# dpeerlab/sctools

Hardware: AMD Instinct MI355X
Metric: Hamming pair-comparisons/sec, 737K 10x whitelist all-pairs, 1-8 GPUs (higher is better)
Workload: dtype i32; 1 GPU; config 2: 737280-barcode all-pairs TwoBit Hamming histogram + summary; barcodes=737280, barcode_length=16, pairs=271790530560, scheme=spectral, parallelism=single GPU

## Files before the change

sctools_amd/csrc/spectral.hip:

```cpp
#include <string.h>

#include <algorithm>
#include <vector>
#include <type_traits>

#include <mutex>

#include <hipcub/hipcub.hpp>

#include "sct_common.h"
#include "spectral.h"
#include "spectral_seed.h"
#ifdef SCT_SEED_MX_VARIANT
#include "spectral_seed_mx.h"
#endif

namespace sct_spectral {
namespace {

using Cols = Columns<kLoBits>;
constexpr int kLo = Cols::kLo;
constexpr int kHiBits = Cols::kHiBits;
constexpr int kRegGroups = 2;
constexpr int kMaxOrder = 1 << 16;

template <int N>
__device__ __forceinline__ void wht(int32_t* x) {
#pragma unroll
  for (int h = 1; h < N; h <<= 1)
#pragma unroll
    for (int i = 0; i < N; ++i)
      if (!(i & h)) {
        const int32_t a = x[i], b = x[i | h];
        x[i] = a + b;
        x[i | h] = a - b;
      }
}

constexpr int kSortWGs = 128;
constexpr int kSortThreads = 1024;

__global__ __launch_bounds__(kSortThreads) void column_hist_wg_kernel(const uint64_t* __restrict__ codes, int64_t n,
                                                                      uint32_t* __restrict__ H) {
  __shared__ uint32_t h[kLo];
  for (int c = threadIdx.x; c < kLo; c += kSortThreads) h[c] = 0;
  __syncthreads();
  int64_t b, e;
  wg_range(n, b, e);
  for (int64_t i = b + threadIdx.x; i < e; i += kSortThreads) atomicAdd(&h[codes[i] & (kLo - 1)], 1u);
  __syncthreads();
  uint32_t* out = H + (int64_t)blockIdx.x * kLo;
  for (int c = threadIdx.x; c < kLo; c += kSortThreads) out[c] = h[c];
}

__global__ __launch_bounds__(256) void column_prefix_kernel(uint32_t* __restrict__ H, int wgs,
                                                            uint32_t* __restrict__ m) {
  const int c = blockIdx.x * 256 + threadIdx.x;
  uint32_t run = 0;
#pragma unroll 8
  for (int g = 0; g < wgs; ++g) {
    const uint32_t v = H[(int64_t)g * kLo + c];
    H[(int64_t)g * kLo + c] = run;
    run += v;
  }
  m[c] = run;
}

__global__ __launch_bounds__(1024) void column_scan16_kernel(const uint32_t* __restrict__ m,
                                                             uint32_t* __restrict__ off,
                                                             uint32_t* __restrict__ gofs) {
  __shared__ uint32_t wsum[2][16];
  const int t = threadIdx.x, lane = t & 63, wave = t >> 6;
  uint32_t v[16];
#pragma unroll
  for (int k = 0; k < 4; ++k) {
    const uint4 q = reinterpret_cast<const uint4*>(m)[t * 4 + k];
    v[4 * k] = q.x;
    v[4 * k + 1] = q.y;
    v[4 * k + 2] = q.z;
    v[4 * k + 3] = q.w;
  }
  uint32_t s = 0, sg = 0;
#pragma unroll
  for (int k = 0; k < 16; ++k) {
    s += v[k];
    sg += (v[k] + 31) / 32;
  }
  uint32_t is = s, isg = sg;
#pragma unroll
  for (int d = 1; d < 64; d <<= 1) {
    const uint32_t a = __shfl_up(is, d), ag = __shfl_up(isg, d);
    if (lane >= d) {
      is += a;
      isg += ag;
    }
  }
  if (lane == 63) {
    wsum[0][wave] = is;
    wsum[1][wave] = isg;
  }
  __syncthreads();
  uint32_t base = 0, baseg = 0;
  for (int w = 0; w < wave; ++w) {
    base += wsum[0][w];
    baseg += wsum[1][w];
  }
  uint32_t run = base + is - s, rung = baseg + isg - sg;
  uint32_t o[16], og[16];
#pragma unroll
  for (int k = 0; k < 16; ++k) {
    o[k] = run;
    og[k] = rung;
    run += v[k];
    rung += (v[k] + 31) / 32;
  }
#pragma unroll
  for (int k = 0; k < 4; ++k) {
    reinterpret_cast<uint4*>(off)[t * 4 + k] = make_uint4(o[4 * k], o[4 * k + 1], o[4 * k + 2], o[4 * k + 3]);
    reinterpret_cast<uint4*>(gofs)[t * 4 + k] = make_uint4(og[4 * k], og[4 * k + 1], og[4 * k + 2], og[4 * k + 3]);
  }
  if (t == 1023) {
    off[kLo] = run;
    gofs[kLo] = rung;
  }
}

__global__ __launch_bounds__(kSortThreads) void column_scatter_wg_kernel(const uint64_t* __restrict__ codes,
                                                                         int64_t n,
                                                                         const uint32_t* __restrict__ H,
                                                                         const uint32_t* __restrict__ off,
                                                                         uint32_t* __restrict__ hi) {
  __shared__ uint32_t cur[kLo];
  const uint32_t* pre = H + (int64_t)blockIdx.x * kLo;
  for (int c = threadIdx.x; c < kLo; c += kSortThreads) cur[c] = off[c] + pre[c];
  __syncthreads();
  int64_t b, e;
  wg_range(n, b, e);
  for (int64_t i = b + threadIdx.x; i < e; i += kSortThreads) {
    const uint64_t x = codes[i];
    hi[atomicAdd(&cur[x & (kLo - 1)], 1u)] = (uint32_t)(x >> kLoBits);
  }
}

__global__ void planes_kernel(const uint32_t* __restrict__ hi, const uint32_t* __restrict__ off,
                              const uint32_t* __restrict__ gofs, int64_t max_groups,
                              uint32_t* __restrict__ planes) {
  const int64_t g = blockIdx.x * (int64_t)blockDim.x + threadIdx.x;
  if (g >= (int64_t)gofs[kLo]) return;
  int a = 0, b = kLo;
  while (b - a > 1) {
    const int m = (a + b) >> 1;
    if (gofs[m] <= (uint32_t)g) a = m;
    else b = m;
  }
  const uint32_t first = off[a] + 32u * ((uint32_t)g - gofs[a]);
  const uint32_t last = min(first + 32u, off[a + 1]);
  uint32_t p[kHiBits];
#pragma unroll
  for (int k = 0; k < kHiBits; ++k) p[k] = 0;
  for (uint32_t i = first; i < last; ++i) {
    const uint32_t h = hi[i], bit = 1u << (i - first);
#pragma unroll
    for (int k = 0; k < kHiBits; ++k) p[k] |= (h >> k) & 1u ? bit : 0u;
  }
  store_planes<Cols>(planes, g, p);
}

typedef unsigned v4u __attribute__((ext_vector_type(4)));

template <typename T>
struct Chunk {
  static constexpr int kVals = 16 / sizeof(T);
  static constexpr int kLog = sizeof(T) == 1 ? 4 : (sizeof(T) == 2 ? 3 : 2);
  static constexpr int kPerThread = 64 / kVals;
};

template <typename T>
__device__ __forceinline__ int column_pos(int c) {
  constexpr int L = Chunk<T>::kLog;
  return (c & ((1 << L) - 1)) | (((c >> 4) & 255) << L) | (((c >> L) & ((16 >> L) - 1)) << (L + 8)) |
         ((c >> 12) << 12);
}


template <typename T>
__device__ __forceinline__ void seed_body(const uint32_t* __restrict__ planes, const uint32_t* __restrict__ gofs,
                                          const uint32_t* __restrict__ off, int z0, int z1, T* __restrict__ buf) {
  constexpr int NT = 256;
  constexpr int P = 4 / sizeof(T);
  constexpr int V = Chunk<T>::kVals;
  __shared__ uint32_t stage[(kWalk / P) * NT];
  const int tid = threadIdx.x;
  const int c0 = blockIdx.x * NT, c = c0 + tid;
  const int m = (int)(off[c + 1] - off[c]);
  const uint32_t g0 = gofs[c];
  const int ng = (int)(gofs[c + 1] - g0);
  int wng = ng;
#pragma unroll
  for (int s = 32; s; s >>= 1) wng = max(wng, __shfl_xor(wng, s));
  uint32_t pr[kRegGroups][kHiBits];
#pragma unroll
  for (int g = 0; g < kRegGroups; ++g)
    if (g < ng) {
      load_planes<Cols>(planes, (int64_t)g0 + g, pr[g]);
    } else {
#pragma unroll
      for (int k = 0; k < kHiBits; ++k) pr[g][k] = 0u;
    }
  {
    const int ph = (blockIdx.x + blockIdx.y) % 3;
    if (ph >= 1) __builtin_amdgcn_s_sleep(24);
    if (ph == 2) __builtin_amdgcn_s_sleep(24);
  }
  const int za = z0 & ~(kWalk - 1);
  const int nwalks = (z1 - za + kWalk - 1) / kWalk;
  for (int wk = blockIdx.y; wk < nwalks; wk += gridDim.y) {
    const int zblk = za + wk * kWalk;
    int acc[kWalk];
    auto walk = [&](const uint32_t* p, auto first) {
      uint32_t x = 0;
#pragma unroll
      for (int k = kWalkBits; k < kHiBits; ++k)
        if ((zblk >> k) & 1) x ^= p[k];
      if constexpr (decltype(first)::value) acc[0] = __popc(x);
      else acc[0] += __popc(x);
#pragma unroll
      for (int i = 1; i < kWalk; ++i) {
        x ^= p[ctz_c(i)];
        if constexpr (decltype(first)::value) acc[gray(i)] = __popc(x);
        else acc[gray(i)] += __popc(x);
      }
    };
    walk(pr[0], std::true_type());
#pragma unroll
    for (int g = 1; g < kRegGroups; ++g)
      if (g < wng) walk(pr[g], std::false_type());
    for (int g = kRegGroups; g < wng; ++g) {
      uint32_t p[kHiBits];
      if (g < ng) {
        load_planes<Cols>(planes, (int64_t)g0 + g, p);
      } else {
#pragma unroll
        for (int k = 0; k < kHiBits; ++k) p[k] = 0u;
      }
      walk(p, std::false_type());
    }
    {
      __syncthreads();
      auto sidx = [](int row, int col) { return row * 256 + (col ^ (((col >> 6) & 3) << 2)); };
#pragma unroll
      for (int r = 0; r < kWalk / P; ++r) {
        uint32_t w = 0;
#pragma unroll
        for (int j = 0; j < P; ++j)
          w |= ((uint32_t)(m - 2 * acc[r * P + j]) & (0xFFFFFFFFu >> (32 - 8 * sizeof(T)))) << (8 * sizeof(T) * j);
        stage[sidx(r, tid)] = w;
      }
      __syncthreads();
      constexpr int kBlocks = (kWalk / P) * (256 / V);
#pragma unroll
      for (int r = 0; r < kBlocks / 256; ++r) {
        const int b = tid + 256 * r, row = b / (256 / V), cb = (b % (256 / V)) * V;
        uint32_t d[V];
#pragma unroll
        for (int k = 0; k < V; k += 4) {
          const uint4 v = *reinterpret_cast<const uint4*>(stage + sidx(row, cb + k));
          d[k] = v.x;
          d[k + 1] = v.y;
          d[k + 2] = v.z;
          d[k + 3] = v.w;
        }
        uint32_t out[P][4];
        if constexpr (P == 2) {
#pragma unroll
          for (int k = 0; k < 4; ++k) {
            out[0][k] = __builtin_amdgcn_perm(d[2 * k + 1], d[2 * k], 0x05040100u);
            out[1][k] = __builtin_amdgcn_perm(d[2 * k + 1], d[2 * k], 0x07060302u);
          }
        } else {
#pragma unroll
          for (int k = 0; k < 4; ++k) out[0][k] = d[k];
        }
#pragma unroll
        for (int j = 0; j < P; ++j) {
          const int z = zblk + row * P + j;
          if (z < z0 || z >= z1) continue;
          *reinterpret_cast<uint4*>(buf + (int64_t)(z - z0) * kLo + column_pos<T>(c0 + cb)) =
              make_uint4(out[j][0], out[j][1], out[j][2], out[j][3]);
        }
      }
    }
  }
}

__global__ __launch_bounds__(256) __attribute__((amdgpu_waves_per_eu(5))) void seed_sm_kernel(
    const uint32_t* __restrict__ planes, const uint32_t* __restrict__ gofs, const uint32_t* __restrict__ off, int z0,
    int z1, int8_t* __restrict__ buf, int lp) {
  seed_sm_body<Cols>(planes, gofs, off, z0, z1, buf, lp);
}

#ifdef SCT_SEED_MX_VARIANT
__global__ __launch_bounds__(64 * kMxWaves) void seed_mx_kernel(const uint32_t* __restrict__ planes,
                                                                const uint32_t* __restrict__ gofs,
                                                                const uint32_t* __restrict__ off, int z0, int z1,
                                                                int8_t* __restrict__ buf, int sb) {
  seed_mx_body<Cols>(planes, gofs, off, z0, z1, buf, sb);
}
#endif

template <typename T>
__global__ __launch_bounds__(256) void seed_kernel(const uint32_t* __restrict__ planes,
                                                   const uint32_t* __restrict__ gofs,
                                                   const uint32_t* __restrict__ off, int z0, int z1,
                                                   T* __restrict__ buf) {
  seed_body<T>(planes, gofs, off, z0, z1, buf);
}

__device__ __forceinline__ int swz(int e) {
  return e ^ (((e >> 6) & 1) << 2) ^ (((e >> 5) & 1) << 3) ^ (((e >> 10) & 1) << 4);
}

__device__ __forceinline__ void lane_butterfly32(int32_t& a, int32_t& b) {
  const auto r = __builtin_amdgcn_permlane32_swap((unsigned)a, (unsigned)b, false, false);
  a = (int32_t)(r[0] + r[1]);
  b = (int32_t)(r[0] - r[1]);
}
__device__ __forceinline__ void lane_butterfly16(int32_t& a, int32_t& b) {
  const auto r = __builtin_amdgcn_permlane16_swap((unsigned)a, (unsigned)b, false, false);
  a = (int32_t)(r[0] + r[1]);
  b = (int32_t)(r[0] - r[1]);
}

template <typename T>
__global__ __launch_bounds__(256) void tile_kernel(const T* __restrict__ buf, int z0, int nslices,
                                                   unsigned long long* __restrict__ counts,
                                                   unsigned long long add_n,
                                                   const unsigned long long* __restrict__ sumsq) {
  static_assert(sizeof(T) >= 2, "int8 seeds take tile_reg_kernel");
  __shared__ int32_t lds[kLo];
  __shared__ unsigned long long bins_lo[17], bins_hi[17];
  constexpr int V = Chunk<T>::kVals, L = Chunk<T>::kLog;
  const int tid = threadIdx.x, lane = tid & 63, wave = tid >> 6;
  if (tid < 17) bins_lo[tid] = bins_hi[tid] = 0;
  const int t2 = (lane & 15) | ((lane >> 4) << 10) | (wave << 12);
  const int wt_thread = digit_weight((uint32_t)lane | ((uint32_t)wave << 12));
  for (int s = blockIdx.x; s < nslices; s += gridDim.x) {
    const T* row = buf + (int64_t)s * kLo;
    int32_t x[64];
#pragma unroll
    for (int j = 0; j < Chunk<T>::kPerThread; ++j) {
      const v4u v = __builtin_nontemporal_load(reinterpret_cast<const v4u*>(row + tid * V + (j << (L + 8))));
      const T* e = reinterpret_cast<const T*>(&v);
#pragma unroll
      for (int r = 0; r < V; ++r) x[j * V + r] = e[r];
    }
    wht<64>(x);
    __syncthreads();
#pragma unroll
    for (int q = 0; q < 64; q += 4)
      *reinterpret_cast<int4*>(lds + swz((q & 15) | (tid << 4) | ((q >> 4) << 12))) =
          make_int4(x[q], x[q + 1], x[q + 2], x[q + 3]);
    __syncthreads();
    const int a2 = swz(t2);
#pragma unroll
    for (int q = 0; q < 64; ++q) x[q] = lds[a2 ^ swz(q << 4)];
    wht<64>(x);
#pragma unroll
    for (int q = 0; q < 64; ++q)
      if (!(q & 2)) lane_butterfly32(x[q], x[q | 2]);
#pragma unroll
    for (int q = 0; q < 64; ++q)
      if (!(q & 1)) lane_butterfly16(x[q], x[q | 1]);
    unsigned long long acc[4] = {0, 0, 0, 0};
#pragma unroll
    for (int q = 0; q < 64; ++q)
      acc[digit_weight_c((uint32_t)(q & 3)) + digit_weight_c((uint32_t)(q >> 2))] +=
          (unsigned long long)((int64_t)x[q] * x[q]);
    const int w0 = digit_weight((uint32_t)(z0 + s)) + wt_thread;
#pragma unroll
    for (int k = 0; k < 4; ++k) {
      if (acc[k] & 0xFFFFFFFFull) atomicAdd(&bins_lo[w0 + k], acc[k] & 0xFFFFFFFFull);
      if (acc[k] >> 32) atomicAdd(&bins_hi[w0 + k], acc[k] >> 32);
    }
  }
  __syncthreads();
  if (tid < 17) add_weight_sum(counts, tid, bins_lo[tid], bins_hi[tid]);
  add_job_constants(counts, add_n, sumsq);
}

typedef int v4i_t __attribute__((ext_vector_type(4)));
typedef short v2s_t __attribute__((ext_vector_type(2)));

typedef int v16i_t __attribute__((ext_vector_type(16)));
constexpr unsigned kChainMaxM = 125;
template <bool Chain>
__global__ __launch_bounds__(256) __attribute__((amdgpu_waves_per_eu(3))) void tile_reg_kernel(
    const int8_t* __restrict__ buf, const uint16_t* __restrict__ order, int z0, int nslices,
    unsigned long long* __restrict__ counts, unsigned long long add_n, const unsigned long long* __restrict__ sumsq) {
  __shared__ unsigned long long bins[17];
  const int tid = threadIdx.x, lane = tid & 63, wave = __builtin_amdgcn_readfirstlane(tid >> 6);
  if (tid < 17) bins[tid] = 0;
  __syncthreads();
  v4i_t H[2][2];
#pragma unroll
  for (int d = 0; d < 4; ++d) {
    uint32_t v = 0;
#pragma unroll
    for (int r = 0; r < 4; ++r) {
      const int row = lane & 31, col = 16 * (lane >> 5) + 4 * d + r;
      v |= ((__popc(row & col) & 1) ? 0xFFu : 0x01u) << (8 * r);
    }
    H[0][0][d] = H[0][1][d] = H[1][0][d] = (int)v;
    H[1][1][d] = (int)(v ^ 0xFEFEFEFEu);
  }
  v4i_t H64[2][2];
  if constexpr (Chain) {
#pragma unroll
    for (int d = 0; d < 4; ++d) {
      const uint32_t v = ((uint32_t)H[0][0][d] << 6) & 0xC0C0C0C0u;
      H64[0][0][d] = H64[0][1][d] = H64[1][0][d] = (int)v;
      H64[1][1][d] = (int)(v ^ 0x80808080u);
    }
  }
  const int wt_thread = digit_weight((uint32_t)lane);
  const int lane_off = 16 * (lane >> 5) + 32 * ((lane >> 3) & 1) + 64 * (lane & 3) + 256 * ((lane >> 4) & 1) +
                       512 * ((lane >> 2) & 1);
  const int gw = blockIdx.x * 4 + wave, GW = gridDim.x * 4;
  const int ub = (int)((int64_t)nslices * gw / GW), ue = (int)((int64_t)nslices * (gw + 1) / GW);
  unsigned long long accA[4] = {0, 0, 0, 0}, accB[4] = {0, 0, 0, 0}, accB2[4] = {0, 0, 0, 0};
  int cur_w = -1;
  auto flush = [&]() {
#pragma unroll
    for (int k = 0; k < 4; ++k) {
      if (accA[k]) atomicAdd(&bins[cur_w + wt_thread + k], accA[k]);
      const unsigned long long b = 4 * (accB[k] + accB2[k]) - accA[k];
      if (b) atomicAdd(&bins[cur_w + wt_thread + k + 1], b);
      accA[k] = 0;
      accB[k] = 0;
      accB2[k] = 0;
    }
  };
  auto load_plane = [&](int sl, int R, v4i_t* dst) {
    const int8_t* p = buf + ((int64_t)sl * kLo + 4096 * R) + lane_off;
#pragma unroll
    for (int k = 0; k < 4; ++k)
      dst[k] = __builtin_nontemporal_load(reinterpret_cast<const v4i_t*>(p + 1024 * k));
  };
  auto stage2 = [&](const v4i_t* Bl, const v4i_t* Bh, auto nt_c, auto chain_c, unsigned long long* acc,
                    unsigned long long* acc2) {
    constexpr int nt = decltype(nt_c)::value;
    v16i_t c[2];
#pragma unroll
    for (int t = 0; t < 2; ++t)
#pragma unroll
      for (int i = 0; i < 16; ++i) c[t][i] = 0;
    if constexpr (decltype(chain_c)::value) {
      v4i_t Bh4[2];
#pragma unroll
      for (int ks = 0; ks < 2; ++ks)
#pragma unroll
        for (int d = 0; d < 4; ++d) Bh4[ks][d] = (int)(((uint32_t)Bh[ks][d] << 2) & 0xFCFCFCFCu);
#pragma unroll
      for (int ks = 0; ks < 2; ++ks)
#pragma unroll
        for (int t = 0; t < 2; ++t)
          c[t] = __builtin_amdgcn_mfma_i32_32x32x32_i8(H64[t][ks], Bh4[ks], c[t], 0, 0, 0);
    } else {
#pragma unroll
      for (int ks = 0; ks < 2; ++ks)
#pragma unroll
        for (int t = 0; t < 2; ++t) c[t] = __builtin_amdgcn_mfma_i32_32x32x32_i8(H[t][ks], Bh[ks], c[t], 0, 0, 0);
#pragma unroll
      for (int t = 0; t < 2; ++t)
#pragma unroll
        for (int i = 0; i < 16; ++i) c[t][i] <<= 8;
    }
#pragma unroll
    for (int ks = 0; ks < 2; ++ks)
#pragma unroll
      for (int t = 0; t < 2; ++t) c[t] = __builtin_amdgcn_mfma_i32_32x32x32_i8(H[t][ks], Bl[ks], c[t], 0, 0, 0);
#pragma unroll
    for (int i = 0; i < 16; ++i) {
      constexpr int w0 = digit_weight_c((uint32_t)nt), w1 = digit_weight_c((uint32_t)(nt | 2));
      const int wi = digit_weight_c((uint32_t)(i & 3)) + digit_weight_c((uint32_t)(i >> 2));
#ifdef SCT_TILE_SQ_ABL
      acc[wi + w0] ^= (uint32_t)c[0][i];
      acc2[wi + w1] ^= (uint32_t)c[1][i];
#else
      acc[wi + w0] += (unsigned long long)((int64_t)c[0][i] * c[0][i]);
      acc2[wi + w1] += (unsigned long long)((int64_t)c[1][i] * c[1][i]);
#endif
    }
  };
  auto split16 = [&](const uint32_t* pr, v4i_t& Bl, v4i_t& Bh) {
#pragma unroll
    for (int d = 0; d < 4; ++d) {
      Bl[d] = (int)(__builtin_amdgcn_perm(pr[2 * d + 1], pr[2 * d], 0x06040200u) ^ 0x80808080u);
      Bh[d] = (int)__builtin_amdgcn_perm(pr[2 * d + 1], pr[2 * d], 0x07050301u);
    }
  };
  auto pairs16 = [&](const v16i_t& c1, uint32_t* pr) {
#pragma unroll
    for (int k = 0; k < 8; ++k)
      pr[k] = __builtin_amdgcn_perm((uint32_t)c1[2 * k + 1], (uint32_t)c1[2 * k], 0x05040100u);
  };
  auto slice_at = [&](int u) { return order ? ((u & ~(kMaxOrder - 1)) | (int)order[u & (kMaxOrder - 1)]) : u; };
  v4i_t dn[4];
  int s_next = ub < ue ? slice_at(ub) : 0;
  if (ub < ue) load_plane(s_next, 0, dn);
  for (int u = ub; u < ue; ++u) {
    const int s = s_next;
    const bool more = u + 1 < ue;
    if (more) s_next = slice_at(u + 1);
    const int wz = digit_weight((uint32_t)(z0 + s));
    if (wz != cur_w) {
      if (cur_w >= 0) flush();
      cur_w = wz;
    }
    uint32_t csp[2][2][8];
#pragma unroll
    for (int nt = 0; nt < 2; ++nt)
#pragma unroll
      for (int mt = 0; mt < 2; ++mt)
#pragma unroll
        for (int k = 0; k < 8; ++k) csp[nt][mt][k] = 0xFE80FE80u;
#pragma unroll 1
    for (int R = 0; R < 4; ++R) {
      v4i_t d[4];
#pragma unroll
      for (int k = 0; k < 4; ++k) d[k] = dn[k];
      if (R < 3 || more) load_plane(R < 3 ? s : s_next, R < 3 ? R + 1 : 0, dn);
      auto ntile = [&](auto nt_c) {
        constexpr int nt = decltype(nt_c)::value;
        v16i_t c1[2];
#pragma unroll
        for (int mt = 0; mt < 2; ++mt)
#pragma unroll
          for (int i = 0; i < 16; ++i) c1[mt][i] = 128;
#pragma unroll
        for (int ks = 0; ks < 2; ++ks)
#pragma unroll
          for (int mt = 0; mt < 2; ++mt)
            c1[mt] = __builtin_amdgcn_mfma_i32_32x32x32_i8(d[2 * mt + ks], H[nt][ks], c1[mt], 0, 0, 0);
        v4i_t Bl[2], Bh[2];
#pragma unroll
        for (int mt = 0; mt < 2; ++mt) {
          uint32_t pr[8];
          pairs16(c1[mt], pr);
#pragma unroll
          for (int k = 0; k < 8; ++k)
            csp[nt][mt][k] = __builtin_bit_cast(uint32_t, __builtin_bit_cast(v2s_t, csp[nt][mt][k]) +
                                                              __builtin_bit_cast(v2s_t, pr[k]));
          split16(pr, Bl[mt], Bh[mt]);
        }
        stage2(Bl, Bh, nt_c, std::bool_constant<Chain>(), accB, Chain ? accB : accB2);
        __builtin_amdgcn_sched_barrier(0);
      };
      ntile(std::integral_constant<int, 0>());
      ntile(std::integral_constant<int, 1>());
    }
    v4i_t Bl[2], Bh[2];
    split16(csp[0][0], Bl[0], Bh[0]);
    split16(csp[0][1], Bl[1], Bh[1]);
    stage2(Bl, Bh, std::integral_constant<int, 0>(), std::false_type(), accA, accA);
    split16(csp[1][0], Bl[0], Bh[0]);
    split16(csp[1][1], Bl[1], Bh[1]);
    stage2(Bl, Bh, std::integral_constant<int, 1>(), std::false_type(), accA, accA);
  }
  if (cur_w >= 0) flush();
  __syncthreads();
  if (tid < 17) add_weight_sum64(counts, tid, bins[tid]);
  add_job_constants(counts, add_n, sumsq);
}

__global__ void low32_kernel(const uint64_t* __restrict__ codes, int64_t n, uint32_t* __restrict__ out) {
  for (int64_t i = blockIdx.x * (int64_t)blockDim.x + threadIdx.x; i < n; i += (int64_t)gridDim.x * blockDim.x)
    out[i] = (uint32_t)codes[i];
}

__global__ __launch_bounds__(256) void sumsq_kernel(const uint32_t* __restrict__ sorted, int64_t n,
                                                    unsigned long long* __restrict__ out) {
  unsigned long long acc = 0;
  for (int64_t i = blockIdx.x * (int64_t)blockDim.x + threadIdx.x; i < n; i += (int64_t)gridDim.x * blockDim.x) {
    const uint32_t v = sorted[i];
    int64_t r = 0;
    if (i > 0 && sorted[i - 1] == v) {
      int64_t a = 0, b = i - 1;
      while (a < b) {
        const int64_t m = (a + b) >> 1;
        if (sorted[m] < v) a = m + 1;
        else b = m;
      }
      r = i - a;
    }
    acc += 2 * (unsigned long long)r + 1;
  }
#pragma unroll
  for (int s = 32; s; s >>= 1) acc += __shfl_xor(acc, s);
  if ((threadIdx.x & 63) == 0 && acc) atomicAdd(out, acc);
}

__global__ __launch_bounds__(256) void probe_kernel(const uint64_t* __restrict__ codes, int64_t n,
                                                    uint32_t* __restrict__ cnt14, uint32_t* __restrict__ cnt16,
                                                    unsigned long long* __restrict__ out) {
  unsigned long long o = 0;
  for (int64_t i = blockIdx.x * (int64_t)blockDim.x + threadIdx.x; i < n; i += (int64_t)gridDim.x * blockDim.x) {
    const uint64_t x = codes[i];
    o |= x;
    atomicAdd(&cnt14[x & (kLo - 1)], 1u);
    atomicAdd(&cnt16[x & 0xFFFFu], 1u);
  }
#pragma unroll
  for (int s = 32; s; s >>= 1) o |= __shfl_xor(o, s);
  if ((threadIdx.x & 63) == 0 && o) atomicOr(out, o);
}
constexpr int64_t kProbeHistMin = 1 << 17;
__global__ __launch_bounds__(kSortThreads) void probe_hist14_kernel(const uint64_t* __restrict__ codes, int64_t n,
                                                                    uint32_t* __restrict__ H,
                                                                    unsigned long long* __restrict__ out) {
  __shared__ uint32_t h[kLo];
  for (int c = threadIdx.x; c < kLo; c += kSortThreads) h[c] = 0;
  __syncthreads();
  int64_t b, e;
  wg_range(n, b, e);
  unsigned long long o = 0;
  for (int64_t i = b + threadIdx.x; i < e; i += kSortThreads) {
    const uint64_t x = codes[i];
    o |= x;
    atomicAdd(&h[x & (kLo - 1)], 1u);
  }
#pragma unroll
  for (int s = 32; s; s >>= 1) o |= __shfl_xor(o, s);
  if ((threadIdx.x & 63) == 0 && o) atomicOr(out, o);
  __syncthreads();
  uint32_t* row = H + (int64_t)blockIdx.x * kLo;
  for (int c = threadIdx.x; c < kLo; c += kSortThreads) row[c] = h[c];
}

__global__ __launch_bounds__(256) void probe_max14_kernel(const uint32_t* __restrict__ H, int wgs,
                                                          unsigned long long* __restrict__ out) {
  const int c = blockIdx.x * 256 + threadIdx.x;
  uint32_t m = 0;
#pragma unroll 8
  for (int g = 0; g < wgs; ++g) m += H[(int64_t)g * kLo + c];
#pragma unroll
  for (int s = 32; s; s >>= 1) m = max(m, (uint32_t)__shfl_xor(m, s));
  if ((threadIdx.x & 63) == 0 && m) atomicMax(out + 1, (unsigned long long)m);
}

__global__ __launch_bounds__(256) void probe_max_kernel(const uint32_t* __restrict__ cnt14,
                                                        const uint32_t* __restrict__ cnt16,
                                                        unsigned long long* __restrict__ out) {
  const int c = blockIdx.x * 256 + threadIdx.x;
  unsigned m14 = c < kLo ? cnt14[c] : 0u, m16 = cnt16[c];
#pragma unroll
  for (int s = 32; s; s >>= 1) {
    m14 = max(m14, (unsigned)__shfl_xor(m14, s));
    m16 = max(m16, (unsigned)__shfl_xor(m16, s));
  }
  if ((threadIdx.x & 63) == 0) {
    if (m14) atomicMax(out + 1, (unsigned long long)m14);
    if (m16) atomicMax(out + 2, (unsigned long long)m16);
  }
}

template <typename T>
int launch_seed(State& st, T* buf, int z0, int z1, hipStream_t s) {
  if constexpr (sizeof(T) == 1) {
#ifdef SCT_SEED_MX_VARIANT
    return launch_seed_mx<Cols>(seed_mx_kernel, st, buf, z0, z1, s);
#else
    return launch_seed_sm<Cols>(seed_sm_kernel, st, buf, z0, z1, s);
#endif
  } else {
    const int walks = (z1 - (z0 & ~(kWalk - 1)) + kWalk - 1) / kWalk;
    const int per_wg = std::max(1, std::min(kSeedWalks, walks / 64));
    const dim3 sgrid(kLo / 256, (unsigned)((walks + per_wg - 1) / per_wg));
    hipLaunchKernelGGL(seed_kernel<T>, sgrid, dim3(256), 0, s, st.d_planes, st.d_gofs, st.d_off, z0, z1, buf);
    SCT_LAUNCH_CHECK();
    return SCT_OK;
  }
}

template <typename T>
int launch_tile(State& st, int z0, int z1, unsigned long long* counts, hipStream_t s, unsigned long long add_n = 0) {
  T* buf = reinterpret_cast<T*>(st.d_buf);
  if constexpr (sizeof(T) == 1) {
    const int ns = z1 - z0;
    const uint16_t* order = ((ns & (ns - 1)) == 0 && z0 % ns == 0) ? st.d_order + std::min(ns, kMaxOrder) : nullptr;
    const dim3 rgrid((unsigned)std::max(1, std::min(st.grid * st.tile_wgs, (z1 - z0 + 3) / 4)));
    hipLaunchKernelGGL(st.tile_chain ? tile_reg_kernel<true> : tile_reg_kernel<false>, rgrid, dim3(256), 0, s, buf,
                       order, z0, z1 - z0, counts, add_n, st.sumsq_ptr());
  } else {
    const dim3 grid((unsigned)std::min(st.grid * 2, z1 - z0));
    hipLaunchKernelGGL(tile_kernel<T>, grid, dim3(256), 0, s, buf, z0, z1 - z0, counts, add_n,
                       st.sumsq_ptr());
  }
  SCT_LAUNCH_CHECK();
  return SCT_OK;
}

template <typename T>
int launch_chunk(State& st, int z0, int z1, unsigned long long* counts, hipStream_t s, unsigned long long add_n) {
  return launch_seed_tile(
      st, s, [&] { return launch_seed<T>(st, reinterpret_cast<T*>(st.d_buf), z0, z1, s); },
      [&] { return launch_tile<T>(st, z0, z1, counts, s, add_n); });
}

template <typename T>
int time_chunk(State& st, int z0, int z1, unsigned long long* counts, int repeats, hipStream_t s,
               double* seed_ms, double* tile_ms) {
  return time_seed_tile(
      st, repeats, s, [&] { return launch_seed<T>(st, reinterpret_cast<T*>(st.d_buf), z0, z1, s); },
      [&] { return launch_tile<T>(st, z0, z1, counts, s); }, seed_ms, tile_ms);
}

}

struct Workspace {
  int device = -1;
  bool busy = false;
  bool release = false;
  bool order_ready = false;
  void* p[W_NSLOTS] = {};
  size_t cap[W_NSLOTS] = {};
  bool arena = false;
  uint8_t* base = nullptr;
  size_t size = 0, used = 0;
  std::vector<void*> extra;
};

namespace {
std::mutex g_ws_mu;
Workspace* g_ws[64] = {};

void ws_free(Workspace* ws) {
  if (ws->arena) {
    if (ws->base) (void)hipFree(ws->base);
    for (void* q : ws->extra) (void)hipFree(q);
  } else {
    for (int k = 0; k < W_NSLOTS; ++k)
      if (ws->p[k]) (void)hipFree(ws->p[k]);
  }
  delete ws;
}
}

Workspace* ws_arena(size_t bytes) {
  auto* ws = new Workspace();
  ws->arena = true;
  ws->busy = true;
  if (hipGetDevice(&ws->device) != hipSuccess || hipMalloc((void**)&ws->base, bytes) != hipSuccess) {
    (void)hipGetLastError();
    ws->base = nullptr;
    bytes = 0;
  }
  ws->size = bytes;
  return ws;
}

Workspace* ws_acquire() {
  if (sct::tune(SCT_TUNE_PLAN_CACHE, 1) == 0) return nullptr;
  int dev = 0;
  if (hipGetDevice(&dev) != hipSuccess || dev < 0 || dev >= 64) return nullptr;
  std::lock_guard<std::mutex> lk(g_ws_mu);
  Workspace*& ws = g_ws[dev];
  if (!ws) {
    ws = new Workspace();
    ws->device = dev;
  }
  if (ws->busy) return nullptr;
  ws->busy = true;
  ws->release = false;
  return ws;
}

void ws_release(Workspace* ws) {
  if (!ws) return;
  if (ws->arena) {
    ws_free(ws);
    return;
  }
  std::lock_guard<std::mutex> lk(g_ws_mu);
  ws->busy = false;
  if (ws->release) {
    g_ws[ws->device] = nullptr;
    ws_free(ws);
  }
}

int ws_get(Workspace* ws, int slot, size_t bytes, void** p) {
  bytes = std::max<size_t>(bytes, 256);
  if (!ws) {
    SCT_HIP(hipMalloc(p, bytes));
    return SCT_OK;
  }
  if (ws->arena) {
    if (ws->cap[slot] < bytes) {
      const size_t at = (ws->used + 255) & ~(size_t)255;
      if (ws->base && at + bytes <= ws->size) {
        ws->p[slot] = ws->base + at;
        ws->used = at + bytes;
      } else {
        void* q = nullptr;
        SCT_HIP(hipMalloc(&q, bytes));
        ws->extra.push_back(q);
        ws->p[slot] = q;
      }
      ws->cap[slot] = bytes;
      if (slot == W_ORDER) ws->order_ready = false;
    }
    *p = ws->p[slot];
    return SCT_OK;
  }
  if (ws->cap[slot] < bytes) {
    if (ws->p[slot]) (void)hipFree(ws->p[slot]);
    ws->p[slot] = nullptr;
    ws->cap[slot] = 0;
    if (slot == W_ORDER) ws->order_ready = false;
    SCT_HIP(hipMalloc(&ws->p[slot], bytes));
    ws->cap[slot] = bytes;
  }
  *p = ws->p[slot];
  return SCT_OK;
}

void ws_put(Workspace* ws, void* p) {
  if (!ws && p) (void)hipFree(p);
}

bool* ws_order_ready(Workspace* ws) { return ws ? &ws->order_ready : nullptr; }

void ws_release_all() {
  std::lock_guard<std::mutex> lk(g_ws_mu);
  for (auto& ws : g_ws) {
    if (!ws) continue;
    if (ws->busy) {
      ws->release = true;
      continue;
    }
    int cur = 0;
    const bool dev_ok = hipGetDevice(&cur) == hipSuccess && hipSetDevice(ws->device) == hipSuccess;
    ws_free(ws);
    if (dev_ok) (void)hipSetDevice(cur);
    ws = nullptr;
  }
}

void note_stream(State& st, hipStream_t s) {
  for (auto& u : st.used)
    if (u.first == s) {
      (void)hipEventRecord(u.second, s);
      return;
    }
  hipEvent_t e = nullptr;
  if (hipEventCreateWithFlags(&e, hipEventDisableTiming) != hipSuccess) return;
  (void)hipEventRecord(e, s);
  st.used.emplace_back(s, e);
}

int make_order_table(State& st) {
  static const std::vector<uint16_t> order = [] {
    std::vector<uint16_t> o(2 * kMaxOrder);
    for (int len = 1; len <= kMaxOrder; len *= 2) {
      int start[10] = {};
      for (int u = 0; u < len; ++u) ++start[digit_weight_c((uint32_t)u) + 1];
      for (int w = 1; w < 10; ++w) start[w] += start[w - 1];
      uint16_t* b = o.data() + len;
      for (int u = 0; u < len; ++u) b[start[digit_weight_c((uint32_t)u)]++] = (uint16_t)u;
    }
    return o;
  }();
  void* p = nullptr;
  if (int rc = ws_get(st.ws, W_ORDER, order.size() * 2, &p); rc != SCT_OK) return rc;
  st.d_order = reinterpret_cast<uint16_t*>(p);
  bool* ready = ws_order_ready(st.ws);
  if (!ready || !*ready) {
    SCT_HIP(hipMemcpy(st.d_order, order.data(), order.size() * 2, hipMemcpyHostToDevice));
    if (ready) *ready = true;
  }
  return SCT_OK;
}

int probe(Workspace* ws, const uint64_t* d_codes, int64_t n, unsigned long long* out) {
  void* p = nullptr;
  constexpr size_t kWords = (size_t)kLo + (1u << 16);
  const bool hist = n >= kProbeHistMin;
  const size_t hbytes = hist ? (size_t)kSortWGs * kLo * 4 : 0;
  if (int rc = ws_get(ws, W_PROBE, hbytes + kWords * 4 + 32, &p); rc != SCT_OK) return rc;
  struct Put {
    Workspace* ws;
    void* p;
    ~Put() { ws_put(ws, p); }
  } put{ws, p};
  uint32_t* H = reinterpret_cast<uint32_t*>(p);
  uint32_t* cnt14 = reinterpret_cast<uint32_t*>(reinterpret_cast<uint8_t*>(p) + hbytes);
  uint32_t* cnt16 = cnt14 + kLo;
  unsigned long long* res = reinterpret_cast<unsigned long long*>(cnt16 + (1u << 16));
  const int blocks = (int)std::max<int64_t>(1, std::min<int64_t>(1024, sct::ceil_div(n, 256)));
  if (hist) {
    SCT_HIP(hipMemsetAsync(res, 0, 32, 0));
    hipLaunchKernelGGL(probe_hist14_kernel, dim3(kSortWGs), dim3(kSortThreads), 0, 0, d_codes, n, H, res);
    SCT_LAUNCH_CHECK();
    hipLaunchKernelGGL(probe_max14_kernel, dim3(kLo / 256), dim3(256), 0, 0, H, kSortWGs, res);
    SCT_LAUNCH_CHECK();
    SCT_HIP(hipMemcpy(out, res, 3 * sizeof(unsigned long long), hipMemcpyDeviceToHost));
    if (out[1] <= 127 && sct::tune(SCT_TUNE_SPECTRAL_COLUMNS, 0) != kLoBits16) return SCT_OK;
  }
  SCT_HIP(hipMemsetAsync(cnt14, 0, kWords * 4 + 32, 0));
  if (n > 0) {
    hipLaunchKernelGGL(probe_kernel, dim3(blocks), dim3(256), 0, 0, d_codes, n, cnt14, cnt16, res);
    SCT_LAUNCH_CHECK();
    hipLaunchKernelGGL(probe_max_kernel, dim3((1u << 16) / 256), dim3(256), 0, 0, cnt14, cnt16, res);
    SCT_LAUNCH_CHECK();
  }
  SCT_HIP(hipMemcpy(out, res, 3 * sizeof(unsigned long long), hipMemcpyDeviceToHost));
  return SCT_OK;
}

int alloc_buf(State& st, int64_t* chunk, int64_t min_chunk, size_t bytes_per_slice) {
  for (;;) {
    const size_t bytes = (size_t)((*chunk + 15) & ~15ll) * bytes_per_slice;
    const int rc = ws_get(st.ws, W_BUF, bytes, &st.d_buf);
    if (rc == SCT_OK) {
      st.buf_bytes = bytes;
      return SCT_OK;
    }
    (void)hipGetLastError();
    if (rc != SCT_E_NOMEM || *chunk / 2 < min_chunk) return rc;
    *chunk /= 2;
  }
}

template <typename K>
static int tile_wgs_per_cu(K kernel) {
  int v = 0;
  if (hipOccupancyMaxActiveBlocksPerMultiprocessor(&v, kernel, 256, 0) != hipSuccess || v <= 0) v = 2;
  return v;
}

int create(State& st, const uint64_t* d_codes, int64_t n, int64_t chunk, int cus, unsigned max14, unsigned max16) {
  st.n = n;
  st.chunk = std::max<int64_t>(kWalk, std::min<int64_t>(chunk, kSlices));
  st.grid = std::max(1, cus);
  if (n < 2) return SCT_OK;
  const unsigned maxm = max14;
  const int64_t force = sct::tune(SCT_TUNE_SPECTRAL_COLUMNS, 0);
  if (((maxm > 127 && force != kLoBits) || force == kLoBits16) && max16 <= 127)
    return create16(st, d_codes, n, max16, chunk, cus);
  if (int rc = get_slot(st, W_HI, (size_t)n * 4, &st.d_hi); rc != SCT_OK) return rc;
  if (int rc = get_slot(st, W_OFF, (size_t)(kLo + 1) * 4, &st.d_off); rc != SCT_OK) return rc;
  if (int rc = get_slot(st, W_CNT, (size_t)2 * kLo * 4, &st.d_cnt); rc != SCT_OK) return rc;
  st.max_m = maxm;
  st.elem_bytes = maxm <= 127 ? 1 : (maxm <= 32767 ? 2 : 4);
  st.chunk = std::min<int64_t>(st.chunk, (int64_t(4) << 30) / ((int64_t)kLo * st.elem_bytes));
  st.tile_chain = st.elem_bytes == 1 && maxm <= kChainMaxM && sct::tune(SCT_TUNE_TILE_CHAIN, 1) != 0;
  static const int per_cu[2] = {tile_wgs_per_cu(tile_reg_kernel<false>), tile_wgs_per_cu(tile_reg_kernel<true>)};
  st.tile_wgs = per_cu[st.tile_chain];
  if (int rc = make_order_table(st); rc != SCT_OK) return rc;
  st.max_groups = sct::ceil_div(n, 32) + kLo;
  if (int rc = get_slot(st, W_GOFS, (size_t)(kLo + 1) * 4, &st.d_gofs); rc != SCT_OK) return rc;
  if (int rc = get_slot(st, W_HIST, (size_t)kSortWGs * kLo * 4, &st.d_hist); rc != SCT_OK) return rc;
  if (int rc = get_slot(st, W_PLANES, (size_t)st.max_groups * Cols::kPlaneWords * 4, &st.d_planes); rc != SCT_OK)
    return rc;
  if (int rc = alloc_buf(st, &st.chunk, std::min<int64_t>(st.chunk, 4096), (size_t)kLo * st.elem_bytes); rc != SCT_OK)
    return rc;
  if (int rc = get_slot(st, W_SUMSQ, sizeof(unsigned long long), &st.d_sumsq); rc != SCT_OK) return rc;
  return SCT_OK;
}

void wait_idle(State& st) {
  for (auto& u : st.used) {
    (void)hipEventSynchronize(u.second);
    (void)hipEventDestroy(u.second);
  }
  st.used.clear();
}

void destroy(State& st) {
  wait_idle(st);
  for (void* p : {(void*)st.d_hi, (void*)st.d_off, (void*)st.d_cnt, (void*)st.d_gofs, (void*)st.d_planes,
                  (void*)st.d_hist, st.d_buf, (void*)st.d_order, (void*)st.d_sumsq, st.d_sumsq_tmp})
    ws_put(st.ws, p);
  ws_release(st.ws);
  st = State();
}

int ensure_sumsq(State& st, const uint64_t* d_codes, hipStream_t s) {
  if (st.sumsq_ready || st.distinct) return SCT_OK;
  size_t tmp = 0;
  SCT_HIP(hipcub::DeviceRadixSort::SortKeys(nullptr, tmp, (const uint32_t*)nullptr, (uint32_t*)nullptr, (int)st.n, 0,
                                            32, s));
  const size_t keys = ((size_t)st.n * 4 + 255) & ~(size_t)255;
  const size_t need = 2 * keys + tmp;
  char* base = reinterpret_cast<char*>(st.d_buf);
  if (need > st.buf_bytes) {
    if (int rc = ws_get(st.ws, W_SUMSQ_TMP, need, &st.d_sumsq_tmp); rc != SCT_OK) return rc;
    base = reinterpret_cast<char*>(st.d_sumsq_tmp);
  }
  uint32_t* k0 = reinterpret_cast<uint32_t*>(base);
  uint32_t* k1 = reinterpret_cast<uint32_t*>(base + keys);
  const int blocks = (int)std::min<int64_t>(2048, sct::ceil_div(st.n, 256));
  hipLaunchKernelGGL(low32_kernel, dim3(blocks), dim3(256), 0, s, d_codes, st.n, k0);
  SCT_LAUNCH_CHECK();
  SCT_HIP(hipcub::DeviceRadixSort::SortKeys(base + 2 * keys, tmp, k0, k1, (int)st.n, 0, 32, s));
  SCT_HIP(hipMemsetAsync(st.d_sumsq, 0, sizeof(unsigned long long), s));
  hipLaunchKernelGGL(sumsq_kernel, dim3(blocks), dim3(256), 0, s, k1, st.n, st.d_sumsq);
  SCT_LAUNCH_CHECK();
  st.sumsq_ready = true;
  return SCT_OK;
}

int build(State& st, const uint64_t* d_codes, hipStream_t s) {
  if (st.n < 2) return SCT_OK;
  if (int rc = ensure_sumsq(st, d_codes, s); rc != SCT_OK) return rc;
  if (st.lo_bits == kLoBits16) return build16(st, d_codes, s);
  hipEvent_t t0 = st.timer ? st.timer->start(s) : nullptr;
  hipLaunchKernelGGL(column_hist_wg_kernel, dim3(kSortWGs), dim3(kSortThreads), 0, s, d_codes, st.n, st.d_hist);
  SCT_LAUNCH_CHECK();
  hipLaunchKernelGGL(column_prefix_kernel, dim3(kLo / 256), dim3(256), 0, s, st.d_hist, kSortWGs, st.d_cnt);
  SCT_LAUNCH_CHECK();
  hipLaunchKernelGGL(column_scan16_kernel, dim3(1), dim3(1024), 0, s, st.d_cnt, st.d_off, st.d_gofs);
  SCT_LAUNCH_CHECK();
  hipLaunchKernelGGL(column_scatter_wg_kernel, dim3(kSortWGs), dim3(kSortThreads), 0, s, d_codes, st.n, st.d_hist,
                     st.d_off, st.d_hi);
  SCT_LAUNCH_CHECK();
  if (st.max_m <= 32 * kPlaneSlots) {
    hipLaunchKernelGGL(planes_slot_kernel<Cols>, dim3(kLo * kPlaneSlots / 256), dim3(256), 0, s, st.d_hi, st.d_off,
                       st.d_gofs, st.d_planes);
  } else {
    hipLaunchKernelGGL(planes_kernel, dim3((unsigned)sct::ceil_div(st.max_groups, 256)), dim3(256), 0, s,
                       st.d_hi, st.d_off, st.d_gofs, st.max_groups, st.d_planes);
  }
  SCT_LAUNCH_CHECK();
  if (st.timer) st.timer->stop(s, t0, sct::LaunchTimer::BUILD);
  return SCT_OK;
}

int count(State& st, int64_t z_begin, int64_t z_end, unsigned long long* d_counts, hipStream_t s) {
  SCT_CHECK(0 <= z_begin && z_begin <= z_end && z_end <= kSlices, "slice range [%lld, %lld)",
            (long long)z_begin, (long long)z_end);
  if (st.n < 2 || z_begin == z_end) return SCT_OK;
  if (st.lo_bits == kLoBits16) return count16(st, z_begin, z_end, d_counts, s);
  for (int64_t z0 = z_begin; z0 < z_end; z0 += st.chunk) {
    const int z1 = (int)std::min<int64_t>(z_end, z0 + st.chunk);
    const unsigned long long add_n = z0 == 0 ? (unsigned long long)st.n : 0ull;
    const int rc = st.elem_bytes == 1   ? launch_chunk<int8_t>(st, (int)z0, z1, d_counts, s, add_n)
                   : st.elem_bytes == 2 ? launch_chunk<int16_t>(st, (int)z0, z1, d_counts, s, add_n)
                                        : launch_chunk<int32_t>(st, (int)z0, z1, d_counts, s, add_n);
    if (rc != SCT_OK) return rc;
  }
  return SCT_OK;
}

int seed_slices(State& st, int64_t z_begin, int64_t z_end, int8_t* d_out, hipStream_t s) {
  SCT_CHECK(0 <= z_begin && z_begin < z_end && z_end <= kSlices, "seed_slices: slice range [%lld, %lld)",
            (long long)z_begin, (long long)z_end);
  SCT_CHECK(st.n >= 2 && st.lo_bits == kLoBits && st.elem_bytes == 1, "seed_slices: not an int8 plan on 14-bit columns");
  return launch_seed<int8_t>(st, d_out, (int)z_begin, (int)z_end, s);
}

int seed_rows(State& st, int64_t z_begin, int64_t z_end, void* d_out, int64_t out_bytes, hipStream_t s) {
  SCT_CHECK(st.n >= 2, "seed_rows: a plan of fewer than 2 codes has no seed");
  const int64_t slices = st.lo_bits == kLoBits16 ? kSlices16 : kSlices;
  SCT_CHECK(0 <= z_begin && z_begin < z_end && z_end <= slices, "seed_rows: slice range [%lld, %lld) outside [0, %lld)",
            (long long)z_begin, (long long)z_end, (long long)slices);
  const int64_t row = ((int64_t)1 << st.lo_bits) * st.elem_bytes;
  SCT_CHECK(out_bytes == (z_end - z_begin) * row, "seed_rows: %lld bytes for %lld rows of %lld", (long long)out_bytes,
            (long long)(z_end - z_begin), (long long)row);
  const int z0 = (int)z_begin, z1 = (int)z_end;
  if (st.lo_bits == kLoBits16) return seed_rows16(st, z0, z1, static_cast<int8_t*>(d_out), s);
  return st.elem_bytes == 1   ? launch_seed<int8_t>(st, static_cast<int8_t*>(d_out), z0, z1, s)
         : st.elem_bytes == 2 ? launch_seed<int16_t>(st, static_cast<int16_t*>(d_out), z0, z1, s)
                              : launch_seed<int32_t>(st, static_cast<int32_t*>(d_out), z0, z1, s);
}

int time_kernels(State& st, int64_t z_begin, int64_t z_end, unsigned long long* d_counts, int repeats,
                 hipStream_t s, double* seed_ms, double* tile_ms, int64_t* slices) {
  SCT_CHECK(0 <= z_begin && z_begin < z_end && z_end <= kSlices && repeats > 0 && st.n >= 2,
            "time_kernels: empty range or plan");
  if (st.lo_bits == kLoBits16) return time_kernels16(st, z_begin, z_end, d_counts, repeats, s, seed_ms, tile_ms, slices);
  const int z1 = (int)std::min<int64_t>(z_end, z_begin + st.chunk);
  *slices = z1 - z_begin;
  return st.elem_bytes == 1   ? time_chunk<int8_t>(st, (int)z_begin, z1, d_counts, repeats, s, seed_ms, tile_ms)
         : st.elem_bytes == 2 ? time_chunk<int16_t>(st, (int)z_begin, z1, d_counts, repeats, s, seed_ms, tile_ms)
                              : time_chunk<int32_t>(st, (int)z_begin, z1, d_counts, repeats, s, seed_ms, tile_ms);
}

}
```

Before: 155100 billion pairs/s.

## Exploit symmetry in N-tile 1 stage2 to halve MFMAs and reorder stage1

For N-tile 1, where both M-tiles fall in the same weight bin, stage2 now issues only the diagonal MFMAs (t == ks) using a single H operand. It compensates algebraically by doubling the squared terms or summing them into a separate Bn accumulator that flush folds back with a factor of 2. Stage1 for both N-tiles is also hoisted ahead of stage2 behind a sched_barrier, so the MFMA chains can overlap better. The aim is to cut MFMA work in the inner loop. The cost is more live registers for the pr buffers and a correctness dependence on the symmetry identity.

```diff
diff --git a/sctools_amd/csrc/spectral.hip b/sctools_amd/csrc/spectral.hip
--- a/sctools_amd/csrc/spectral.hip
+++ b/sctools_amd/csrc/spectral.hip
@@ -427,18 +427,20 @@
                        512 * ((lane >> 2) & 1);
   const int gw = blockIdx.x * 4 + wave, GW = gridDim.x * 4;
   const int ub = (int)((int64_t)nslices * gw / GW), ue = (int)((int64_t)nslices * (gw + 1) / GW);
-  unsigned long long accA[4] = {0, 0, 0, 0}, accB[4] = {0, 0, 0, 0}, accB2[4] = {0, 0, 0, 0};
+  unsigned long long accA[4] = {0, 0, 0, 0}, accB[4] = {0, 0, 0, 0}, Bn[3] = {0, 0, 0};
   int cur_w = -1;
   auto flush = [&]() {
 #pragma unroll
     for (int k = 0; k < 4; ++k) {
       if (accA[k]) atomicAdd(&bins[cur_w + wt_thread + k], accA[k]);
-      const unsigned long long b = 4 * (accB[k] + accB2[k]) - accA[k];
+      const unsigned long long n1 = k ? 2 * Bn[k - 1] : 0;
+      const unsigned long long b = 4 * (accB[k] + n1) - accA[k];
       if (b) atomicAdd(&bins[cur_w + wt_thread + k + 1], b);
       accA[k] = 0;
       accB[k] = 0;
-      accB2[k] = 0;
-    }
+    }
+#pragma unroll
+    for (int k = 0; k < 3; ++k) Bn[k] = 0;
   };
   auto load_plane = [&](int sl, int R, v4i_t* dst) {
     const int8_t* p = buf + ((int64_t)sl * kLo + 4096 * R) + lane_off;
@@ -446,15 +448,16 @@
     for (int k = 0; k < 4; ++k)
       dst[k] = __builtin_nontemporal_load(reinterpret_cast<const v4i_t*>(p + 1024 * k));
   };
-  auto stage2 = [&](const v4i_t* Bl, const v4i_t* Bh, auto nt_c, auto chain_c, unsigned long long* acc,
-                    unsigned long long* acc2) {
+  auto stage2 = [&](const v4i_t* Bl, const v4i_t* Bh, auto nt_c, auto chain_c, auto sum_c,
+                    unsigned long long* acc) {
     constexpr int nt = decltype(nt_c)::value;
+    constexpr bool chain = decltype(chain_c)::value, half = nt == 1;
     v16i_t c[2];
 #pragma unroll
     for (int t = 0; t < 2; ++t)
 #pragma unroll
       for (int i = 0; i < 16; ++i) c[t][i] = 0;
-    if constexpr (decltype(chain_c)::value) {
+    if constexpr (chain) {
       v4i_t Bh4[2];
 #pragma unroll
       for (int ks = 0; ks < 2; ++ks)
@@ -464,12 +467,15 @@
       for (int ks = 0; ks < 2; ++ks)
 #pragma unroll
         for (int t = 0; t < 2; ++t)
-          c[t] = __builtin_amdgcn_mfma_i32_32x32x32_i8(H64[t][ks], Bh4[ks], c[t], 0, 0, 0);
+          if (!half || t == ks)
+            c[t] = __builtin_amdgcn_mfma_i32_32x32x32_i8(half ? H64[0][0] : H64[t][ks], Bh4[ks], c[t], 0, 0, 0);
     } else {
 #pragma unroll
       for (int ks = 0; ks < 2; ++ks)
 #pragma unroll
-        for (int t = 0; t < 2; ++t) c[t] = __builtin_amdgcn_mfma_i32_32x32x32_i8(H[t][ks], Bh[ks], c[t], 0, 0, 0);
+        for (int t = 0; t < 2; ++t)
+          if (!half || t == ks)
+            c[t] = __builtin_amdgcn_mfma_i32_32x32x32_i8(half ? H[0][0] : H[t][ks], Bh[ks], c[t], 0, 0, 0);
 #pragma unroll
       for (int t = 0; t < 2; ++t)
 #pragma unroll
@@ -478,17 +484,21 @@
 #pragma unroll
     for (int ks = 0; ks < 2; ++ks)
 #pragma unroll
-      for (int t = 0; t < 2; ++t) c[t] = __builtin_amdgcn_mfma_i32_32x32x32_i8(H[t][ks], Bl[ks], c[t], 0, 0, 0);
+      for (int t = 0; t < 2; ++t)
+        if (!half || t == ks)
+          c[t] = __builtin_amdgcn_mfma_i32_32x32x32_i8(half ? H[0][0] : H[t][ks], Bl[ks], c[t], 0, 0, 0);
 #pragma unroll
     for (int i = 0; i < 16; ++i) {
       constexpr int w0 = digit_weight_c((uint32_t)nt), w1 = digit_weight_c((uint32_t)(nt | 2));
+      static_assert(!half || (w0 == 1 && w1 == 1), "N-tile 1: both M-tiles in one bin");
+      constexpr bool sum = half && decltype(sum_c)::value, dbl = half && !sum;
       const int wi = digit_weight_c((uint32_t)(i & 3)) + digit_weight_c((uint32_t)(i >> 2));
 #ifdef SCT_TILE_SQ_ABL
-      acc[wi + w0] ^= (uint32_t)c[0][i];
-      acc2[wi + w1] ^= (uint32_t)c[1][i];
+      acc[wi + (sum ? 0 : w0)] ^= (uint32_t)c[0][i];
+      acc[wi + (sum ? 0 : w1)] ^= (uint32_t)c[1][i];
 #else
-      acc[wi + w0] += (unsigned long long)((int64_t)c[0][i] * c[0][i]);
-      acc2[wi + w1] += (unsigned long long)((int64_t)c[1][i] * c[1][i]);
+      acc[wi + (sum ? 0 : w0)] += (unsigned long long)((int64_t)(dbl ? 2 * c[0][i] : c[0][i]) * c[0][i]);
+      acc[wi + (sum ? 0 : w1)] += (unsigned long long)((int64_t)(dbl ? 2 * c[1][i] : c[1][i]) * c[1][i]);
 #endif
     }
   };
@@ -530,42 +540,49 @@
 #pragma unroll
       for (int k = 0; k < 4; ++k) d[k] = dn[k];
       if (R < 3 || more) load_plane(R < 3 ? s : s_next, R < 3 ? R + 1 : 0, dn);
+      uint32_t pr[2][2][8];
+      auto stage1 = [&](auto nt_c) {
+        constexpr int nt = decltype(nt_c)::value;
+        v16i_t c1[2];
+#pragma unroll
+        for (int mt = 0; mt < 2; ++mt)
+#pragma unroll
+          for (int i = 0; i < 16; ++i) c1[mt][i] = 128;
+#pragma unroll
+        for (int ks = 0; ks < 2; ++ks)
+#pragma unroll
+          for (int mt = 0; mt < 2; ++mt)
+            c1[mt] = __builtin_amdgcn_mfma_i32_32x32x32_i8(d[2 * mt + ks], H[nt][ks], c1[mt], 0, 0, 0);
+#pragma unroll
+        for (int mt = 0; mt < 2; ++mt) {
+          pairs16(c1[mt], pr[nt][mt]);
+#pragma unroll
+          for (int k = 0; k < 8; ++k)
+            csp[nt][mt][k] = __builtin_bit_cast(uint32_t, __builtin_bit_cast(v2s_t, csp[nt][mt][k]) +
+                                                              __builtin_bit_cast(v2s_t, pr[nt][mt][k]));
+        }
+      };
       auto ntile = [&](auto nt_c) {
         constexpr int nt = decltype(nt_c)::value;
-        v16i_t c1[2];
-#pragma unroll
-        for (int mt = 0; mt < 2; ++mt)
-#pragma unroll
-          for (int i = 0; i < 16; ++i) c1[mt][i] = 128;
-#pragma unroll
-        for (int ks = 0; ks < 2; ++ks)
-#pragma unroll
-          for (int mt = 0; mt < 2; ++mt)
-            c1[mt] = __builtin_amdgcn_mfma_i32_32x32x32_i8(d[2 * mt + ks], H[nt][ks], c1[mt], 0, 0, 0);
         v4i_t Bl[2], Bh[2];
 #pragma unroll
-        for (int mt = 0; mt < 2; ++mt) {
-          uint32_t pr[8];
-          pairs16(c1[mt], pr);
-#pragma unroll
-          for (int k = 0; k < 8; ++k)
-            csp[nt][mt][k] = __builtin_bit_cast(uint32_t, __builtin_bit_cast(v2s_t, csp[nt][mt][k]) +
-                                                              __builtin_bit_cast(v2s_t, pr[k]));
-          split16(pr, Bl[mt], Bh[mt]);
-        }
-        stage2(Bl, Bh, nt_c, std::bool_constant<Chain>(), accB, Chain ? accB : accB2);
+        for (int mt = 0; mt < 2; ++mt) split16(pr[nt][mt], Bl[mt], Bh[mt]);
+        stage2(Bl, Bh, nt_c, std::bool_constant<Chain>(), std::true_type(), nt ? Bn : accB);
         __builtin_amdgcn_sched_barrier(0);
       };
+      stage1(std::integral_constant<int, 1>());
+      stage1(std::integral_constant<int, 0>());
+      __builtin_amdgcn_sched_barrier(0);
       ntile(std::integral_constant<int, 0>());
       ntile(std::integral_constant<int, 1>());
     }
     v4i_t Bl[2], Bh[2];
     split16(csp[0][0], Bl[0], Bh[0]);
     split16(csp[0][1], Bl[1], Bh[1]);
-    stage2(Bl, Bh, std::integral_constant<int, 0>(), std::false_type(), accA, accA);
+    stage2(Bl, Bh, std::integral_constant<int, 0>(), std::false_type(), std::false_type(), accA);
     split16(csp[1][0], Bl[0], Bh[0]);
     split16(csp[1][1], Bl[1], Bh[1]);
-    stage2(Bl, Bh, std::integral_constant<int, 1>(), std::false_type(), accA, accA);
+    stage2(Bl, Bh, std::integral_constant<int, 1>(), std::false_type(), std::false_type(), accA);
   }
   if (cur_w >= 0) flush();
   __syncthreads();
```

New measurement: 159300 billion pairs/s (median of 6 runs). 2.7% higher.
